# RajeshRk18/exacto

Measured on AMD Instinct MI355X. Metric: ciphertext muls/sec (bfv_mul_and_relin), higher is better.
Workload: dtype u64; 1 GPU; bfv_mul_and_relin, BASELINE configs[2]; ring_degree=4096, ct_limbs=3, limb_bits=60, plain_modulus=65537, gadget_base=65536, gadget_digits=12, batch_per_gpu=1024, global_batch=1024, parallelism=batch-shard x1

## Files before the change

### exacto_amd/csrc/ks32.hip

```cpp
#include "exacto_internal.hpp"
#include "ks32_dev.hpp"

#include <algorithm>

namespace exacto {


template <int LOGN, typename DT, int FORM>
__global__ void __launch_bounds__((1 << LOGN) / 16)
ks32_digit_ntt_kernel(const DT* __restrict__ D16, uint32_t* __restrict__ DS, int G, int S,
                      const Prime32* __restrict__ primes) {
    constexpr int N = 1 << LOGN, T = N / 16;
    __shared__ uint32_t lds[N];
    const int tid = threadIdx.x;
    const uint32_t b = blockIdx.x;
    const int s = (int)(b % (uint32_t)S);
    const long ig = b / (uint32_t)S;
    const Prime32& P = primes[s];
    const DT* src = D16 + ig * N;
    uint32_t x[16];
    constexpr bool SIN = FORM == F32_LAZY && sizeof(DT) == 2;
#pragma unroll
    for (int k = 0; k < 16; ++k) {
        const int d = src[tid + k * T];
// ... 46 lines not shown
    __syncthreads();
    for (int w = 128; w > 0; w >>= 1) {
        if ((int)threadIdx.x < w) part[threadIdx.x] += part[threadIdx.x + w];
        __syncthreads();
    }
    if (threadIdx.x == 0) out[row] = part[0];
}

__device__ __forceinline__ uint32_t red_s64(long long x, const Prime32& P) {
    const uint32_t p = P.p;
    const uint32_t hu = (uint32_t)((unsigned long long)x >> 32) ^ 0x80000000u;
    const uint32_t a = red32(shoup32(hu, P.c32, P.c32s, p), p);
    const uint32_t b = red32(red32((uint32_t)x, 2 * p), p);
    return red32(red32(a + b, p) + P.k63, p);
}

__device__ __forceinline__ uint32_t red_s64_lz(long long x, const Prime32& P) {
    const uint32_t p = P.p;
    const uint32_t hu = (uint32_t)((unsigned long long)x >> 32) ^ 0x80000000u;
    const uint32_t a = red32(shoup32(hu, P.c32, P.c32s, p), p);
    const uint32_t lo = (uint32_t)x;
    const uint32_t b = lo - (lo >> 30) * p;
    const uint32_t s = a + b + P.k63;
    return min(s, s - 2 * p);
}

__device__ __forceinline__ long long red_s64_lazy(long long x, const Prime32& P) {
    const uint32_t hu = (uint32_t)((unsigned long long)x >> 32) ^ 0x80000000u;
    const uint32_t a = shoup32(hu, P.c32, P.c32s, P.p);
    return (long long)((unsigned long long)a + (uint32_t)x + P.k63);
}

constexpr int KS_LS = 64;
template <int CLB, int NW, int RUN, bool LZ = false>
__global__ void __launch_bounds__(NW * 64)
ks32_mac_kernel(const int* __restrict__ DS, const int* __restrict__ RS, uint32_t* __restrict__ U,
                int G, int CL, int S, int items, int n, const Prime32* __restrict__ primes) {
    extern __shared__ int kl[];
    constexpr int IG = 4 * NW;
    const int lane = threadIdx.x & (KS_LS - 1);
    const int wave = __builtin_amdgcn_readfirstlane(threadIdx.x / KS_LS);
    const int nb = n / KS_LS;
    const int jb = blockIdx.x % nb;
    const int s = (blockIdx.x / nb) % S;
    const int cl0 = (blockIdx.x / (nb * S)) * CLB;
    const int j = jb * KS_LS + lane;
    const Prime32& P = primes[s];
    for (int rr = wave; rr < G * CLB; rr += NW) {
        const int g = rr / CLB, c = rr - g * CLB;
        kl[rr * KS_LS + lane] = RS[(((long)g * CL + cl0 + c) * S + s) * n + jb * KS_LS + lane];
    }
    __syncthreads();
    const int it_end = min(items, (int)(blockIdx.y + 1) * IG);
    for (int it = blockIdx.y * IG + wave; it < it_end; it += NW) {
        const int* dp = DS + ((long)it * G * S + s) * n + j;
        long long acc[CLB];
#pragma unroll
        for (int c = 0; c < CLB; ++c) acc[c] = 0;
        for (int g0 = 0; g0 < G; g0 += RUN) {
            int d[RUN];
#pragma unroll
            for (int e = 0; e < RUN; ++e) d[e] = dp[(long)min(g0 + e, G - 1) * S * n];
#pragma unroll
            for (int e = 0; e < RUN; ++e) d[e] = g0 + e < G ? d[e] : 0;
#pragma unroll
            for (int e = 0; e < RUN; ++e) {
                const int* kg = kl + (min(g0 + e, G - 1) * CLB) * KS_LS + lane;
#pragma unroll
                for (int c = 0; c < CLB; ++c) acc[c] += (long long)d[e] * kg[c * KS_LS];
            }
            if (g0 + RUN < G) {
#pragma unroll
                for (int c = 0; c < CLB; ++c) acc[c] = red_s64_lazy(acc[c], P);
            }
        }
#pragma unroll
        for (int c = 0; c < CLB; ++c)
            U[(((long)it * CL + cl0 + c) * S + s) * n + j] = LZ ? red_s64_lz(acc[c], P) : red_s64(acc[c], P);
    }
}

template <int LOGN, int S, bool LAZY, bool FPC>
__global__ void __launch_bounds__((1 << LOGN) / 16)
ks32_crt_kernel(const uint32_t* __restrict__ U, u64* __restrict__ R, long r_stride, int L,
                const Ks32Tables* __restrict__ KT, const Prime32* __restrict__ primes,
                const PrimeConst* __restrict__ qprimes) {
    constexpr int N = 1 << LOGN, T = N / 16;
    __shared__ uint32_t lds[N];
    const int tid = threadIdx.x;
    const uint32_t b = blockIdx.x;
    u64 x[16];
    ks32_crt_values<LOGN, S, LAZY, FPC>(x, U, R, r_stride, L, b, lds, tid, KT, primes, qprimes);
    const uint32_t CL = 2 * L;
    const long item = b / CL;
    const __amdgpu_buffer_rsrc_t rd = poly_rsrc(R + item * r_stride + (long)(b - (uint32_t)item * CL) * N, N * 8);
#pragma unroll
    for (int k = 0; k < 16; ++k) buf_st64(rd, x[k], tid * 8, k * T * 8);
}

template <typename OT, typename IT>
__global__ void __launch_bounds__(256)
ks32_digit_sum_kernel(const IT* __restrict__ D, int npairs, const int* __restrict__ term_start,
                      const CombineTerm* __restrict__ terms, OT* __restrict__ out, int d, int gu, int n,
                      int nsh) {
    const uint32_t row = blockIdx.x >> nsh;
    const int j = (int)(blockIdx.x & ((1u << nsh) - 1)) * 2048 + 8 * threadIdx.x;
    const uint32_t g = row % (uint32_t)gu;
    const uint32_t ik = row / (uint32_t)gu;
    const int k = (int)(ik % (uint32_t)d);
    const long item = ik / (uint32_t)d;
    int acc[8] = {0, 0, 0, 0, 0, 0, 0, 0};
    for (int t = term_start[k]; t < term_start[k + 1]; ++t) {
        const IT* src = D + ((item * npairs + terms[t].pair) * gu + g) * (long)n + j;
        if constexpr (sizeof(IT) == 2) {
            const uint4 w = *reinterpret_cast<const uint4*>(src);
            const uint32_t v[4] = {w.x, w.y, w.z, w.w};
#pragma unroll
            for (int h = 0; h < 4; ++h) {
                acc[2 * h] += (int)(int16_t)(v[h] & 0xFFFF);
                acc[2 * h + 1] += (int)(int16_t)(v[h] >> 16);
            }
        } else {
            const uint2 w = *reinterpret_cast<const uint2*>(src);
            const uint32_t v[2] = {w.x, w.y};
#pragma unroll
            for (int h = 0; h < 8; ++h) acc[h] += (int)(int8_t)(v[h >> 2] >> (8 * (h & 3)));
        }
    }
    if constexpr (sizeof(OT) == 2) {
        uint4 o;
        uint32_t* op = &o.x;
#pragma unroll
// ... 8 lines not shown


#define FORM_SWITCH(form, CALL)                          \
    switch (form) {                                      \
        case F32_LAZY: CALL(F32_LAZY); break;            \
        case F32_NARROW: CALL(F32_NARROW); break;        \
        default: CALL(F32_WIDE); break;                  \
    }

template <int LOGN>
static void ks32_launch_digits(const void* D, bool wide, uint32_t* DS, int items, int G, int S, const Prime32* primes,
                               int form, hipStream_t st) {
    const dim3 grid((unsigned)((long)items * G * S)), block((1 << LOGN) / 16);
#define DIG_(F_)                                                                                                \
    do {                                                                                                        \
        if (wide)                                                                                               \
            EXACTO_LAUNCH((ks32_digit_ntt_kernel<LOGN, int32_t, F_>), grid, block, 0, st, (const int32_t*)D, \
                               DS, G, S, primes);                                                               \
        else                                                                                                    \
            EXACTO_LAUNCH((ks32_digit_ntt_kernel<LOGN, int16_t, F_>), grid, block, 0, st, (const int16_t*)D, \
                               DS, G, S, primes);                                                               \
    } while (0)
    FORM_SWITCH(form, DIG_)
#undef DIG_
}

template <int LOGN>
static void ks32_launch_key(const u64* K, uint32_t* RS, long rows, int L, int S, const Prime32* primes,
                            const PrimeConst* qprimes, int form, hipStream_t st) {
#define KEY_(F_) EXACTO_LAUNCH((ks32_key_kernel<LOGN, F_>), dim3((unsigned)(rows * S)), dim3((1 << LOGN) / 16), 0, \
                                    st, K, RS, L, S, primes, qprimes)
    FORM_SWITCH(form, KEY_)
#undef KEY_
}

template <int LOGN, bool LAZY>
static void ks32_launch_crt(const uint32_t* U, u64* R, long r_stride, int items, int L, int S, const Ks32Tables* KT,
                            const Prime32* primes, const PrimeConst* qprimes, hipStream_t st, bool fpc) {
    const dim3 grid((unsigned)((long)items * 2 * L)), block((1 << LOGN) / 16);
#define CRT_(S_, F_) EXACTO_LAUNCH((ks32_crt_kernel<LOGN, S_, LAZY, F_>), grid, block, 0, st, U, R, r_stride, L, KT, \
                                   primes, qprimes)
    if (S == 2) {
        if (fpc) CRT_(2, true); else CRT_(2, false);
    } else if (S == 3) {
        if (fpc) CRT_(3, true); else CRT_(3, false);
    } else {
        if (fpc) CRT_(4, true); else CRT_(4, false);
    }
#undef CRT_
}

#define KS32_SWITCH(logn, CALL)                  \
    switch (logn) {                              \
        case 10: CALL(10); break;                \
        case 11: CALL(11); break;                \
        case 12: CALL(12); break;                \
        case 13: CALL(13); break;                \
        case 14: CALL(14); break;                \
        default: break;                          \
    }

void ks32_digits(const int16_t* D16, uint32_t* DS, int items, int G, int S, int logn, const Prime32* primes, int form,
                 hipStream_t st) {
    if (items <= 0) return;
#define CALL(L_) ks32_launch_digits<L_>(D16, false, DS, items, G, S, primes, form, st)
    KS32_SWITCH(logn, CALL)
#undef CALL
}

void ks32_digits32(const int32_t* D, uint32_t* DS, int items, int G, int S, int logn, const Prime32* primes, int form,
                   hipStream_t st) {
    if (items <= 0) return;
#define CALL(L_) ks32_launch_digits<L_>(D, true, DS, items, G, S, primes, form, st)
    KS32_SWITCH(logn, CALL)
#undef CALL
}

void ks32_key(const u64* K, uint32_t* RS, long rows, int L, int S, int logn, const Prime32* primes,
              const PrimeConst* qprimes, int form, hipStream_t st) {
    if (rows <= 0) return;
#define CALL(L_) ks32_launch_key<L_>(K, RS, rows, L, S, primes, qprimes, form, st)
    KS32_SWITCH(logn, CALL)
#undef CALL
}

void ks32_key_norms(const u64* K, u64* out, long rows, int L, int n, const PrimeConst* qprimes, hipStream_t st) {
    if (rows <= 0) return;
    EXACTO_LAUNCH(ks32_key_norm_kernel, dim3((unsigned)rows), dim3(256), 0, st, K, out, L, n, qprimes);
}

void ks32_mac(const uint32_t* DS, const uint32_t* RS, uint32_t* U, int items, int G, int L, int S, int n,
              const Prime32* primes, int mac_form, hipStream_t st) {
    if (items <= 0) return;
    const int CL = 2 * L;
    int CLB = CL;
    while (CLB > 1 && (CL % CLB != 0 || (size_t)G * CLB * KS_LS * sizeof(int) > 65536)) --CLB;
    const size_t lds = (size_t)G * CLB * KS_LS * sizeof(int);
    const int NW = lds > 32768 ? 8 : 4;
    const dim3 grid((unsigned)((n / KS_LS) * S * (CL / CLB)), (unsigned)((items + 4 * NW - 1) / (4 * NW)));
    const int* ds = reinterpret_cast<const int*>(DS);
    const int* rs = reinterpret_cast<const int*>(RS);
#define MAC_(C_, W_, R_, Z_) EXACTO_LAUNCH((ks32_mac_kernel<C_, W_, R_, Z_>), grid, dim3(W_ * 64), lds, st, ds, rs, U, G, CL, S, items, n, primes)
#define MAC(C_)                                                  \
    do {                                                         \
        if (mac_form == 2) { if (NW == 8) MAC_(C_, 8, 12, true); else MAC_(C_, 4, 12, true); } \
        else if (mac_form == 1) { if (NW == 8) MAC_(C_, 8, 12, false); else MAC_(C_, 4, 12, false); } \
        else { if (NW == 8) MAC_(C_, 8, 7, false); else MAC_(C_, 4, 7, false); }          \
    } while (0)
    switch (CLB) {
        case 8: MAC(8); break;
        case 6: MAC(6); break;
        case 4: MAC(4); break;
        case 3: MAC(3); break;
        case 2: MAC(2); break;
        default: MAC(1); break;
    }
#undef MAC
#undef MAC_
}

void ks32_digit_sum(const void* D, bool in8, int npairs, const int* term_start, const CombineTerm* terms, void* out,
                    bool wide, int items, int d, int gu, int n, hipStream_t st) {
    const long rows = (long)items * d * gu;
    if (rows <= 0) return;
    const int nb = n >= 2048 ? n / 2048 : 1;
    const dim3 grid((unsigned)(rows * nb)), block(n >= 2048 ? 256 : n / 8);
    const int nsh = __builtin_ctz((unsigned)nb);
#define DSUM_(OT, IT) EXACTO_LAUNCH((ks32_digit_sum_kernel<OT, IT>), grid, block, 0, st, (const IT*)D, npairs, \
                                         term_start, terms, (OT*)out, d, gu, n, nsh)
    if (wide) {
        if (in8) DSUM_(int32_t, int8_t); else DSUM_(int32_t, int16_t);
    } else {
        if (in8) DSUM_(int16_t, int8_t); else DSUM_(int16_t, int16_t);
    }
#undef DSUM_
}

void ks32_crt(const uint32_t* U, u64* R, long r_stride, int items, int L, int S, int logn, const Ks32Tables* KT,
              const Prime32* primes, const PrimeConst* qprimes, int form, hipStream_t st, bool fpc) {
    if (items <= 0) return;
    fpc = fpc && (S <= 3 || form != F32_WIDE);
#define CALL(L_)                                                                                                \
    do {                                                                                                        \
        if (form == F32_LAZY) ks32_launch_crt<L_, true>(U, R, r_stride, items, L, S, KT, primes, qprimes, st, fpc); \
        else ks32_launch_crt<L_, false>(U, R, r_stride, items, L, S, KT, primes, qprimes, st, fpc);                \
    } while (0)
    KS32_SWITCH(logn, CALL)
#undef CALL
}

}
```

### exacto_amd/csrc/context.hip

```cpp
#include <algorithm>
#include <cxxabi.h>
#include <dlfcn.h>
#include <chrono>
#include <condition_variable>
#include <cmath>
#include <cstdio>
#include <cstdlib>
#include <cstring>
#include <functional>
#include <map>
#include <memory>
#include <mutex>
#include <set>
#include <string>
#include <thread>
#include <vector>

#include "../../include/exacto_hip.h"
#include "exacto_internal.hpp"

using namespace exacto;

thread_local const void* exacto::g_last_kernel = nullptr;

// ... 1098 lines not shown
        if (hipEventRecord(rec.b, c->stream) == hipSuccess) c->recs.push_back(rec);
    }
};

static int run_ntt(exacto_ctx* c, const NttBatch& nb, long count, bool inverse) {
    if (count <= 0) return 0;
    ProfScope ps(c, inverse ? PK_INV : PK_FWD, (u64)count, ((nb.src16 ? 2.0 : 8.0) + 8.0) * c->n * (double)count);
    bool lazy = true, near60 = c->ntt_asm;
    int qbits = 0;
    for (int t = nb.prime_base; t < nb.prime_base + nb.period; ++t) {
        lazy &= c->primes[t] < (1ull << 60);
        near60 &= c->primes[t] < (1ull << 60) && c->primes[t] > (1ull << 60) - (1ull << 32);
        qbits = std::max(qbits, 64 - __builtin_clzll(c->primes[t]));
    }
    launch_ntt(nb, (int)count, c->logn, inverse, lazy, c->d_primes, c->stream, near60, near60 && c->ntt_asm_inv, qbits);
    CHECK_LAUNCH();
    return 0;
}

static int run_ntt_fwd2(exacto_ctx* c, const NttBatch& nb1, long count1, const NttBatch& nb2, long count2) {
    bool near60 = c->ntt_asm && !nb1.src16 && !nb2.src16;
    for (u64 q : c->primes) near60 &= q < (1ull << 60) && q > (1ull << 60) - (1ull << 32);
    if (near60 && count1 > 0 && count2 > 0) {
        ProfScope ps(c, PK_FWD, (u64)(count1 + count2), 16.0 * c->n * (double)(count1 + count2));
        if (launch_ntt_fwd2(nb1, (int)count1, nb2, (int)count2, c->logn, c->d_primes, c->stream)) {
            CHECK_LAUNCH();
            return 0;
        }
    }
    if (int e = run_ntt(c, nb1, count1, false)) return e;
    return run_ntt(c, nb2, count2, false);
}

static bool tensor_asm(const exacto_ctx* c) {
    bool near60 = c->ntt_asm && c->ntt_asm_inv;
    for (int t = 0; t < c->L + c->K; ++t)
        near60 &= c->primes[t] < (1ull << 60) && c->primes[t] > (1ull << 60) - (1ull << 24);
    return near60;
}

static int run_inv_tensor(exacto_ctx* c, const Operands& o, int cnt, bool p2only = false) {
    const int NP = c->L + c->K;
    bool lazy = true;
    const bool near60 = tensor_asm(c);
    int qbits = 0;
    for (int t = 0; t < NP; ++t) {
        qbits = std::max(qbits, 64 - __builtin_clzll(c->primes[t]));
        lazy &= c->primes[t] < (1ull << 60);
    }
    const double pb = 8.0 * c->n;
    double bytes;
    if (c->tensor_share_d > 0 && c->tensor_share_npairs > 0) {
        const double items = (double)((cnt + c->tensor_share_npairs - 1) / c->tensor_share_npairs);
        const double cts = items * 2.0 * c->tensor_share_d;
        bytes = pb * (c->L * (2.0 * cts + 3.0 * cnt) +
                      c->K * (p2only ? cts + (double)cnt : 2.0 * cts + 3.0 * cnt));
    } else {
        bytes = cnt * (p2only ? pb * (7.0 * c->L + 3.0 * c->K) : pb * 7.0 * NP);
    }
    ProfScope ps(c, PK_TENSOR, (u64)cnt * (p2only ? 3 * c->L + c->K : 3 * NP), bytes);
    launch_inv_tensor(o, c->ws_extP, c->ws_T, cnt, c->logn, c->L, c->K, lazy, c->d_primes, c->stream, near60, p2only,
                      qbits, c->tensor_share_npairs, near60 && c->path != EXACTO_PATH_HPS);
    CHECK_LAUNCH();
    return 0;
}

// ... 282 lines not shown
        if (c->path == EXACTO_PATH_HPS) {
            void* d16p = hps_defer ? (c->ks_defer8 ? (void*)((int8_t*)c->ks_defer + s * (long)guse * n)
                                                   : (void*)(c->ks_defer + s * (long)guse * n))
                                   : nullptr;
            launch_hps_scale(c->ws_T, R, out_stride, ncomp, hps_defer ? nullptr : D, d16p,
                             hps_defer && c->ks_defer8, guse, cnt, n, c->d_crt, c->d_primes, K, c->hps_fast,
                             c->stream);
        } else
            launch_exact_scale(c->ws_T, R, out_stride, ncomp, d16 ? nullptr : D,
                               d16 ? (c->ks_defer ? (c->ks_defer8
                                                         ? (int16_t*)((int8_t*)c->ks_defer + s * (long)guse * n)
                                                         : c->ks_defer + s * (long)guse * n)
                                                  : c->ws_D16)
                                   : nullptr,
                               guse, cnt, n, c->d_crt, c->d_primes, L, K, crt_mode(c),
                               c->stream, c->h_crt.gshift, ps.on, c->ks_defer && c->ks_defer8, c->fp_crt, c->fpq_lim);
        CHECK_LAUNCH();
        }
        if (ps.on) {
            const long item0 = s / ps.npairs;
            const double ib = (double)(cnt / ps.npairs);
            ProfScope pq(c, PK_PSUM_SCALE, (u64)(cnt / ps.npairs) * ps.d,
                         ib * 2.0 * n * 8.0 * (ps.d * (double)(K + L) + (double)ps.npairs * L));
            if (!launch_psum_scale(c->ws_T, c->ws_extP, ps.out + item0 * ps.d * 2 * Ln, cnt / ps.npairs, ps.d, ps.npairs,
                                   ps.term_start, ps.terms, n, c->d_crt, c->d_primes, L, c->stream, ps.fpc,
                                   c->fpq_lim))
                return fail(EXACTO_ERR_HIP, "internal: psum scale not available for these limbs");
            CHECK_LAUNCH();
        }
        NttBatch rb{};
        rb.src = R; rb.src_off = nullptr; rb.src_item_stride = out_stride;
        rb.dst = R; rb.dst_item_stride = out_stride;
        rb.ppi = ncomp * L; rb.prime_base = 0; rb.period = L;
        if (k32) {
            if (!c->ks_defer) {
                {
                    ProfScope pd(c, PK_KS_DIGITS, (u64)cnt * guse * c->S32, 6.0 * n * cnt * guse * c->S32);
                    ks32_digits(c->ws_D16, c->ws_DS, cnt, guse, c->S32, c->logn, c->d_p32, c->ks32_mac_form, c->stream);
                }
                {
                    ProfScope pm(c, PK_KS_MAC, (u64)cnt * c->S32, 4.0 * n * cnt * c->S32 * (guse + 2.0 * L));
                    ks32_mac(c->ws_DS, c->d_rs, c->ws_U, cnt, guse, L, c->S32, n, c->d_p32, c->ks32_mac_form, c->stream);
                }
                {
                    ProfScope pc(c, PK_KS_CRT, (u64)cnt * 2 * L, (double)n * cnt * 2 * L * (4.0 * c->S32 + 16.0));
                    ks32_crt(c->ws_U, R, out_stride, cnt, L, c->S32, c->logn, c->d_kst, c->d_p32, c->d_primes, c->ks32_mac_form,
                             c->stream, c->ks_fpc && c->ks32_fpc_max >= 1);
                }
                CHECK_LAUNCH();
            }
        }
        if (skip_fwd) continue;
        if (int e = run_ntt(c, rb, (long)cnt * ncomp * L, false)) return e;
        if (relin && guse > 0 && !k32) {
            NttBatch db = contiguous(c->ws_D, cnt, (long)guse * L, 0, L, n);
            if (d16) {
                db.src16 = c->ws_D16;
                db.src16_item_stride = (long)guse * n;
            }
            if (int e = run_ntt(c, db, (long)cnt * guse * L, false)) return e;
            if (int e = ensure_rlk_companions(c)) return e;
            {
                ProfScope pm(c, PK_RELIN_MAC, (u64)cnt, 8.0 * n * L * cnt * (4.0 + guse));
                launch_relin_mac(R, out_stride, c->ws_D, c->d_rlk, c->d_rlk_s, guse, R, out_stride, cnt, n, L,
                                 c->d_primes, c->stream);
            }
            CHECK_LAUNCH();
        }
    }
    return 0;
}


static int check_ctx(exacto_ctx* c) {
    if (!c) return invalid_param("null context");
    HIP_TRY(hipSetDevice(c->device));
    return 0;
}

static int ntt_dev(exacto_ctx* c, uint64_t* polys, size_t count, size_t limb, bool inverse) {
    if (int e = check_ctx(c)) return e;
    if (limb >= (size_t)c->L)
        return fail(EXACTO_ERR_DIMENSION_MISMATCH, "dimension mismatch: expected " + std::to_string(c->L) + ", got " +
                                                       std::to_string(limb));
    return run_ntt(c, contiguous(polys, count, 1, (int)limb, 1, c->n), (long)count, inverse);
}
// ... 1129 lines not shown
        if (e) return e;
    } else {
        size_t cap = c->gk_s_cap;
        if (grow(&c->gk_s, &cap, count * sizeof(u64))) return EXACTO_ERR_HIP;
        c->gk_s_cap = cap;
        launch_shoup_companions(gk, c->gk_s, (long)count, n, L, c->d_primes, c->stream);
        CHECK_LAUNCH();
    }
    const size_t C = std::min<size_t>(c->chunk, B);
    if (int e = ensure_workspace(c, C)) return e;
    int nl = 1;
    if (int e = fork_lanes(c, (long)((B + C - 1) / C), C, &nl)) return e;
    LaneJoin join{c, nl};
    for (size_t s0 = 0; s0 < B; s0 += C) {
        const int cnt = (int)std::min(C, B - s0);
        LaneGuard lane(c, (int)((s0 / C) % (size_t)nl));
        const u64* src = ct + s0 * 2 * Ln;
        u64* dst = out + s0 * 2 * Ln;
        NttBatch nb{};
        nb.src = src; nb.src_item_stride = 2 * Ln;
        nb.dst = c->ws_coefQ; nb.dst_item_stride = 2 * Ln;
        nb.ppi = 2 * L; nb.prime_base = 0; nb.period = L;
        if (int e = run_ntt(c, nb, (long)cnt * 2 * L, true)) return e;
        launch_automorph(c->ws_coefQ, 2 * Ln, c->ws_T, 2 * Ln, cnt, 2, n, L, element, c->d_primes, -1, c->stream);
        CHECK_LAUNCH();
        if (k32) {
            launch_decompose(c->ws_T + Ln, 2 * Ln, c->ws_D, guse, cnt, n, c->d_crt, c->d_primes, L, c->stream,
                             c->ws_D16);
            CHECK_LAUNCH();
            launch_rows(c->ws_T + Ln, 2 * Ln, nullptr, 0, Ln, cnt, c->stream);
            CHECK_LAUNCH();
            ks32_digits(c->ws_D16, c->ws_DS, cnt, guse, kb.S, c->logn, kb.d_p32, kb.mac_form, c->stream);
            ks32_mac(c->ws_DS, c->d_gk_rs, c->ws_U, cnt, guse, L, kb.S, n, kb.d_p32, kb.mac_form, c->stream);
            ks32_crt(c->ws_U, c->ws_T, 2 * Ln, cnt, L, kb.S, c->logn, kb.d_kst, kb.d_p32, c->d_primes, kb.mac_form, c->stream,
                     c->ks_fpc && kb.fpc_max >= 1);
            CHECK_LAUNCH();
            NttBatch rb{};
            rb.src = c->ws_T; rb.src_item_stride = 2 * Ln;
            rb.dst = dst; rb.dst_item_stride = 2 * Ln;
            rb.ppi = 2 * L; rb.prime_base = 0; rb.period = L;
            if (int e = run_ntt(c, rb, (long)cnt * 2 * L, false)) return e;
            continue;
        }
        NttBatch c0{};
        c0.src = c->ws_T; c0.src_item_stride = 2 * Ln;
        c0.dst = dst; c0.dst_item_stride = 2 * Ln;
        c0.ppi = L; c0.prime_base = 0; c0.period = L;
        if (int e = run_ntt(c, c0, (long)cnt * L, false)) return e;
        launch_rows(dst + Ln, 2 * Ln, nullptr, 0, Ln, cnt, c->stream);
        launch_decompose(c->ws_T + Ln, 2 * Ln, c->ws_D, guse, cnt, n, c->d_crt, c->d_primes, L, c->stream,
                         d16 ? c->ws_D16 : nullptr);
        CHECK_LAUNCH();
        NttBatch db = contiguous(c->ws_D, cnt, (long)guse * L, 0, L, n);
        if (d16) {
            db.src16 = c->ws_D16;
            db.src16_item_stride = (long)guse * n;
        }
        if (int e = run_ntt(c, db, (long)cnt * guse * L, false)) return e;
        launch_relin_mac(dst, 2 * Ln, c->ws_D, gk, c->gk_s, guse, dst, 2 * Ln, cnt, n, L, c->d_primes, c->stream);
        CHECK_LAUNCH();
    }
    return 0;
}

extern "C" int exacto_gen_galois_key(exacto_ctx* c, const uint64_t* sk, uint64_t element, double sigma,
                                     const uint64_t* key, uint64_t stream, size_t num_keys, uint64_t* gk) {
    if (!c) return invalid_param("null context");
    return host_call(c, {{sk, c->L * poly_bytes(c)}}, num_keys * 2 * c->L * poly_bytes(c), gk,
                     [&](std::vector<u64*>& d, u64* o) {
// ... 1371 lines not shown
```

### exacto_amd/csrc/exacto_internal.hpp

```cpp
#pragma once
#include "arith.hpp"

namespace exacto {

struct NttBatch {
    const u64* src;
    const u64* src_off;
    long src_item_stride;
    u64* dst;
    long dst_item_stride;
    int ppi;
    int prime_base;
    int period;
    const int16_t* src16;
    long src16_item_stride;
    int lazy_out;
};

enum class MulPath : int { Exact = 0, Hps = 1 };

struct CrtTables {
    int L;
    int K;
    int G;
// ... 49 lines not shown

#define EXACTO_KS32_MAXS 4
struct Prime32 {
    uint32_t p;
    uint32_t n_inv, n_inv_s;
    uint32_t last_w, last_ws;
    uint32_t c32, c32s;
    uint32_t k63;
    uint32_t fn_inv, fn_inv_s;
    uint32_t flast_w, flast_ws;
    double inv_p;
    const uint2* tw_fwd;
    const uint2* tw_inv;
};
struct Ks32Tables {
    uint32_t ginv[EXACTO_KS32_MAXS][EXACTO_KS32_MAXS];
    uint32_t ginv_s[EXACTO_KS32_MAXS][EXACTO_KS32_MAXS];
    uint32_t halfP[EXACTO_KS32_MAXS];
    u64 pref_w[EXACTO_MAX_L][EXACTO_KS32_MAXS];
    u64 pref_ws[EXACTO_MAX_L][EXACTO_KS32_MAXS];
    u64 negP[EXACTO_MAX_L];
    uint32_t fpc_c[EXACTO_MAX_L][EXACTO_KS32_MAXS][2];
    uint32_t fpc_n[EXACTO_MAX_L][2];
};
void ks32_digits(const int16_t* D16, uint32_t* DS, int items, int G, int S, int logn, const Prime32* primes,
                 int form, hipStream_t st);
void ks32_digits32(const int32_t* D, uint32_t* DS, int items, int G, int S, int logn, const Prime32* primes,
                   int form, hipStream_t st);
void ks32_key(const u64* K, uint32_t* RS, long rows, int L, int S, int logn, const Prime32* primes,
              const PrimeConst* qprimes, int form, hipStream_t st);
void ks32_key_norms(const u64* K, u64* out, long rows, int L, int n, const PrimeConst* qprimes, hipStream_t st);
void ks32_mac(const uint32_t* DS, const uint32_t* RS, uint32_t* U, int items, int G, int L, int S, int n,
              const Prime32* primes, int mac_form, hipStream_t st);
void ks32_crt(const uint32_t* U, u64* R, long r_stride, int items, int L, int S, int logn, const Ks32Tables* KT,
              const Prime32* primes, const PrimeConst* qprimes, int form, hipStream_t st, bool fpc = false);

struct Operands {
    const u64* a;
    const u64* a_off;
    long a_stride;
    const u64* b;
    const u64* b_off;
    long b_stride;
    const u64* ea;
    const u64* ea_off;
    const u64* eb;
    const u64* eb_off;
};

bool launch_polymul(const u64* A, const u64* B, u64* out, long rows, int period, int logn, const PrimeConst* primes,
                    hipStream_t s);
void launch_mul_inv(const u64* A, const u64* B, u64* out, long rows, int period, int logn, bool lazy, bool asm_inv,
                    const PrimeConst* primes, hipStream_t s);
void launch_inv_tensor(const Operands& op, const u64* extP, u64* T, int items, int logn, int L, int K, bool lazy,
                       const PrimeConst* primes, hipStream_t s, bool asm_inv = false, bool p2only = false,
                       int qbits = 64, int share_np = 0, bool lazy_out = false);
void launch_phase(const u64* ct, int polys, long ct_stride, const u64* sk, u64* out, int items, int n, int L,
                  const PrimeConst* primes, hipStream_t s);
void launch_decrypt_round(const u64* X, u64* out, int items, int n, int L, const CrtTables* ct,
                          const PrimeConst* primes, u64 plain, hipStream_t s);
void launch_dbfv_recompose(const u64* digits, u64* out, int items, int n, int d, u64 base, u64 plain, u64 t,
                           bool scalar, hipStream_t s);
void launch_exact_lift(const u64* coefQ, u64* extP, long rows, int n, const CrtTables* ct,
                       const PrimeConst* primes, int L, int K, int mode, hipStream_t s);
void launch_hps_extend(const u64* coefQ, u64* extP, long rows, int n, const PrimeConst* primes,
                       int K, hipStream_t s);
bool exact_scale_sp_ok(int L, int K, int mode);
void launch_exact_scale(const u64* T, u64* R, long r_stride, int ncomp_r, u64* D, int16_t* D16, int guse,
// ... 90 lines not shown
```

### exacto_amd/csrc/ntt.hip

```cpp
#include "exacto_internal.hpp"
#include "ks32_dev.hpp"
#include "bufmem.hpp"
#include "crt_dev.hpp"

namespace exacto {

#ifndef EXACTO_TW_AS
#define EXACTO_TW_AS 1
#endif
#if EXACTO_TW_AS == 0
typedef const TwPair* TwTab;
#else
typedef const TwPair __attribute__((address_space(EXACTO_TW_AS)))* TwTab;
#endif

__device__ __forceinline__ TwTab tw_table(const TwPair* p) { return (TwTab)p; }

__device__ __forceinline__ TwPair ld_tw(TwTab tab, int i) {
    TwPair t;
    t.w = tab[i].w;
    t.ws = tab[i].ws;
    return t;
}

// ... 591 lines not shown
#undef PIN_SYN
    } else if (nb.src16) {
        const int16_t* s16 = nb.src16 + (long)item * nb.src16_item_stride + (long)(sub / nb.period) * N + tid;
#define PIN_IN16(k) { const i64 d_ = s16[(k) * T]; PIN_SET(k, d_ < 0 ? q + (u64)d_ : (u64)d_) }
        PIN_X16(PIN_IN16)
#undef PIN_IN16
    } else {
        const u64* src = nb.src + (nb.src_off ? (long)nb.src_off[item] : (long)item * nb.src_item_stride) +
                         (long)sub * N;
        const PolyRd rs(src, N * 8);
#define PIN_IN64(k) PIN_SET(k, rs.ld64(tid * 8, (k) * T * 8))
        PIN_X16(PIN_IN64)
#undef PIN_IN64
    }
    if constexpr (PROBE == 2) {
        PIN_EXCHANGE(lds, tid, LOGN - 4, LOGN - 8)
        PIN_EXCHANGE(lds, tid, LOGN - 8, LOGN == 12 ? 0 : 1)
        if constexpr (LOGN == 13) {
            if constexpr (EXACTO_FWD13_LP) EXACTO_XCHG_PIN_LP(tid);
            else PIN_EXCHANGE(lds, tid, 1, 0)
        }
    } else if constexpr (LZO) {
        PIN_FWD_ROUNDS(LOGN, lds, tid, tw_table(P.tw_fwd), make_asmk(q), _LZ)
    } else {
        PIN_FWD_ROUNDS(LOGN, lds, tid, tw_table(P.tw_fwd), make_asmk(q), )
    }
    if constexpr (PROBE == 1) {
        if (nb.dst_item_stride != -7) return;
    }
    const PolyWr rd(dst, N * 8);
#define PIN_OUT(k) rd.st64(PIN_GET(k), tid * 8, fwd_pin_value_of_home<LOGN>(k) * T * 8);
    PIN_X16(PIN_OUT)
#undef PIN_OUT
}


__device__ __forceinline__ u64 barrett_mul_lazy(u64 a, u64 b, const PrimeConst& P) {
    const u64 hi = __umul64hi(a, b), lo = a * b;
    const int s = P.bar_s;
    const u64 xs = (lo >> (s - 1)) | (hi << (65 - s));
    const u64 qhat = ((xs * P.bar_mu) >> (s + 1)) | (__umul64hi(xs, P.bar_mu) << (63 - s));
    return lo - qhat * P.q;
}

__device__ __forceinline__ u64 mulmod_near60(u64 a, u64 b, uint32_t d) {
    constexpr u64 M60 = (1ull << 60) - 1;
    const u64 lo = a * b, hi = __umul64hi(a, b);
    const u64 H = (hi << 4) | (lo >> 60);
    const u64 xl = (lo & M60) + (u64)(uint32_t)H * d;
    const u64 xh = (u64)(uint32_t)(H >> 32) * d + (xl >> 32);
    const u64 H2 = xh >> 28;
    const u64 L2 = ((xh & 0x0FFFFFFFull) << 32) | (uint32_t)xl;
    return L2 + H2 * d;
}

#ifndef EXACTO_MUL_ASM
#define EXACTO_MUL_ASM 1
#endif
template <bool ASM = (EXACTO_MUL_ASM != 0)>
__device__ __forceinline__ void mul2_near60(u64& r0, u64 a0, u64 b0, u64& r1, u64 a1, u64 b1, uint32_t d) {
    if constexpr (ASM) {
        MulNear60Asm<2>::run(r0, r1, a0, b0, a1, b1, d, 16 * d);
    } else {
        r0 = mulmod_near60(a0, b0, d);
        r1 = mulmod_near60(a1, b1, d);
    }
// ... 515 lines not shown
    if (share_np < 8 || items % share_np != 0) share_np = 0;
    const long blocks = (long)items * 3 * (L + K);
    if (blocks == 0) return;
    if (p2only) {
        if (logn == 12) launch_it<12>(op, extP, T, blocks, L, K, lazy, primes, s, true, 1, 64, share_np, lazy_out);
        else if (logn == 13) launch_it<13>(op, extP, T, blocks, L, K, lazy, primes, s, true, 1, 64, share_np, lazy_out);
        return;
    }
    switch (logn) {
        case 4: launch_it<4>(op, extP, T, blocks, L, K, lazy, primes, s); break;
        case 5: launch_it<5>(op, extP, T, blocks, L, K, lazy, primes, s); break;
        case 6: launch_it<6>(op, extP, T, blocks, L, K, lazy, primes, s); break;
        case 7: launch_it<7>(op, extP, T, blocks, L, K, lazy, primes, s); break;
        case 8: launch_it<8>(op, extP, T, blocks, L, K, lazy, primes, s); break;
        case 9: launch_it<9>(op, extP, T, blocks, L, K, lazy, primes, s); break;
        case 10: launch_it<10>(op, extP, T, blocks, L, K, lazy, primes, s, false, 0, qbits, share_np); break;
        case 11: launch_it<11>(op, extP, T, blocks, L, K, lazy, primes, s); break;
        case 12: launch_it<12>(op, extP, T, blocks, L, K, lazy, primes, s, asm_inv, 0, qbits, share_np, lazy_out); break;
        case 13: launch_it<13>(op, extP, T, blocks, L, K, lazy, primes, s, asm_inv, 0, qbits, share_np, lazy_out); break;
        case 14: launch_it<14>(op, extP, T, blocks, L, K, lazy, primes, s); break;
        default: break;
    }
}

bool launch_ntt_fwd2(const NttBatch& nb1, int count1, const NttBatch& nb2, int count2, int logn,
                     const PrimeConst* primes, hipStream_t s) {
    if (count1 <= 0 || count2 <= 0 || (logn != 12 && logn != 13)) return false;
    const dim3 grid((unsigned)(count1 + count2));
    if (logn == 12) EXACTO_LAUNCH((ntt_fwd_pin_kernel<12>), grid, dim3(256), 0, s, nb1, primes, nb2, count1);
    else EXACTO_LAUNCH((ntt_fwd_pin_kernel<13>), grid, dim3(512), 0, s, nb1, primes, nb2, count1);
    return true;
}

void launch_ntt(const NttBatch& nb, int count, int logn, bool inverse, bool lazy, const PrimeConst* primes,
                hipStream_t s, bool asm_fwd, bool asm_inv, int qbits) {
    if (count <= 0) return;
    if (asm_fwd && !inverse && (logn == 12 || logn == 13)) {
        if (nb.lazy_out) {
            if (logn == 12) EXACTO_LAUNCH((ntt_fwd_pin_kernel<12, 0, true>), dim3(count), dim3(256), 0, s, nb, primes);
            else EXACTO_LAUNCH((ntt_fwd_pin_kernel<13, 0, true>), dim3(count), dim3(512), 0, s, nb, primes);
        } else {
            if (logn == 12) EXACTO_LAUNCH((ntt_fwd_pin_kernel<12>), dim3(count), dim3(256), 0, s, nb, primes);
            else EXACTO_LAUNCH((ntt_fwd_pin_kernel<13>), dim3(count), dim3(512), 0, s, nb, primes);
        }
        return;
    }
    if (asm_inv && inverse && (logn == 12 || logn == 13)) {
        if (logn == 12) EXACTO_LAUNCH((ntt_inv_pin_kernel<12>), dim3(count), dim3(256), 0, s, nb, primes);
        else EXACTO_LAUNCH((ntt_inv_pin_kernel<13>), dim3(count), dim3(512), 0, s, nb, primes);
        return;
    }
    if (lazy && (logn == 10 || logn == 12 || logn == 13) && ntt_gen_on()) {
        const dim3 th(1u << (logn - 4));
#define GEN_NTT_(K_, LG_, QB_) EXACTO_LAUNCH((K_<LG_, QB_>), dim3(count), th, 0, s, nb, primes)
        if (inverse) {
            if (logn == 10) { if (gen_small<10>(qbits)) GEN_NTT_(ntt_inv_gen_kernel, 10, 50); else GEN_NTT_(ntt_inv_gen_kernel, 10, 60); }
            else if (logn == 12) { if (gen_small<12>(qbits)) GEN_NTT_(ntt_inv_gen_kernel, 12, 56); else GEN_NTT_(ntt_inv_gen_kernel, 12, 60); }
            else GEN_NTT_(ntt_inv_gen_kernel, 13, 60);
        } else {
            if (logn == 10) { if (gen_small<10>(qbits)) GEN_NTT_(ntt_fwd_gen_kernel, 10, 50); else GEN_NTT_(ntt_fwd_gen_kernel, 10, 60); }
            else if (logn == 12) { if (gen_small<12>(qbits)) GEN_NTT_(ntt_fwd_gen_kernel, 12, 56); else GEN_NTT_(ntt_fwd_gen_kernel, 12, 60); }
            else GEN_NTT_(ntt_fwd_gen_kernel, 13, 60);
        }
#undef GEN_NTT_
        return;
    }
// ... 25 lines not shown
```

Measured before the change: 481,800 bfv_mul_and_relin/s.

## Software-pipeline key-switch MAC digit loads and batch key staging via buffer loads

Restructures the key-switch MAC kernel so each wave double-buffers its digit loads, fetching the next run or item while multiplying the current one, and collapses the item and digit loops into one state machine. Key rows are staged into LDS in batches of nine buffer loads per wave, and all global accesses use buffer resources. The host picks the items-per-block adaptively so the grid has at least twice the CU count of blocks. A specialised single-run variant drops the loop when all digits fit in one run. The change adds register pressure and code complexity in exchange for hiding global memory latency.

Result: no change. 483,200 bfv_mul_and_relin/s (median of 6 runs) (+0.3%).

```diff
diff --git a/exacto_amd/csrc/ks32.hip b/exacto_amd/csrc/ks32.hip
--- a/exacto_amd/csrc/ks32.hip
+++ b/exacto_amd/csrc/ks32.hip
@@ -102,52 +102,88 @@
 }
 
 constexpr int KS_LS = 64;
-template <int CLB, int NW, int RUN, bool LZ = false>
+constexpr unsigned KS_CUS = 256;
+constexpr int KS_SB = 9;
+template <int CLB, int NW, int RUN, bool LZ, bool ONE>
 __global__ void __launch_bounds__(NW * 64)
 ks32_mac_kernel(const int* __restrict__ DS, const int* __restrict__ RS, uint32_t* __restrict__ U,
-                int G, int CL, int S, int items, int n, const Prime32* __restrict__ primes) {
+                int G, int CL, int S, int items, int IG, int n, const Prime32* __restrict__ primes) {
     extern __shared__ int kl[];
-    constexpr int IG = 4 * NW;
     const int lane = threadIdx.x & (KS_LS - 1);
     const int wave = __builtin_amdgcn_readfirstlane(threadIdx.x / KS_LS);
     const int nb = n / KS_LS;
     const int jb = blockIdx.x % nb;
     const int s = (blockIdx.x / nb) % S;
     const int cl0 = (blockIdx.x / (nb * S)) * CLB;
-    const int j = jb * KS_LS + lane;
+    const int j0 = jb * KS_LS;
+    const int voff = lane * 4;
+    const int rowb = n * 4;
     const Prime32& P = primes[s];
-    for (int rr = wave; rr < G * CLB; rr += NW) {
-        const int g = rr / CLB, c = rr - g * CLB;
-        kl[rr * KS_LS + lane] = RS[(((long)g * CL + cl0 + c) * S + s) * n + jb * KS_LS + lane];
+    {
+        const int rows = G * CLB;
+        const __amdgpu_buffer_rsrc_t rk =
+            poly_rsrc(RS + ((long)cl0 * S + s) * n + j0, (((G - 1) * CL + CLB - 1) * S * n + KS_LS) * 4);
+        for (int r0 = wave; r0 < rows; r0 += NW * KS_SB) {
+            int v[KS_SB];
+#pragma unroll
+            for (int k = 0; k < KS_SB; ++k) {
+                const int rr = min(r0 + k * NW, rows - 1);
+                const int g = rr / CLB, c = rr - g * CLB;
+                v[k] = (int)buf_ld32(rk, voff, (g * CL + c) * S * rowb);
+            }
+#pragma unroll
+            for (int k = 0; k < KS_SB; ++k) kl[min(r0 + k * NW, rows - 1) * KS_LS + lane] = v[k];
+        }
     }
     __syncthreads();
     const int it_end = min(items, (int)(blockIdx.y + 1) * IG);
-    for (int it = blockIdx.y * IG + wave; it < it_end; it += NW) {
-        const int* dp = DS + ((long)it * G * S + s) * n + j;
-        long long acc[CLB];
-#pragma unroll
-        for (int c = 0; c < CLB; ++c) acc[c] = 0;
-        for (int g0 = 0; g0 < G; g0 += RUN) {
-            int d[RUN];
-#pragma unroll
-            for (int e = 0; e < RUN; ++e) d[e] = dp[(long)min(g0 + e, G - 1) * S * n];
-#pragma unroll
-            for (int e = 0; e < RUN; ++e) d[e] = g0 + e < G ? d[e] : 0;
-#pragma unroll
-            for (int e = 0; e < RUN; ++e) {
-                const int* kg = kl + (min(g0 + e, G - 1) * CLB) * KS_LS + lane;
-#pragma unroll
-                for (int c = 0; c < CLB; ++c) acc[c] += (long long)d[e] * kg[c * KS_LS];
+    const int it0 = blockIdx.y * IG + wave;
+    if (it0 >= it_end) return;
+    const int dsz = ((G - 1) * S * n + KS_LS) * 4;
+    const int usz = ((CLB - 1) * S * n + KS_LS) * 4;
+    auto load_run = [&](int (&b)[RUN], int it, int g0) {
+        const __amdgpu_buffer_rsrc_t rd = poly_rsrc(DS + ((long)it * G * S + s) * n + j0, dsz);
+#pragma unroll
+        for (int e = 0; e < RUN; ++e) b[e] = (int)buf_ld32(rd, voff, min(g0 + e, G - 1) * S * rowb);
+    };
+    long long acc[CLB];
+#pragma unroll
+    for (int c = 0; c < CLB; ++c) acc[c] = 0;
+    int it = it0, g0 = 0;
+    auto step = [&](int (&cb)[RUN], int (&nb)[RUN]) -> bool {
+        const bool more = !ONE && g0 + RUN < G;
+        const bool last = it + NW >= it_end;
+        const int nit = more || last ? it : it + NW, ng0 = more ? g0 + RUN : 0;
+        load_run(nb, nit, ng0);
+        __builtin_amdgcn_sched_barrier(0);
+        int kofs = lane;
+        asm volatile("" : "+v"(kofs));
+#pragma unroll
+        for (int e = 0; e < RUN; ++e) {
+            const int* kg = kl + min(g0 + e, G - 1) * CLB * KS_LS + kofs;
+            const int d = g0 + e < G ? cb[e] : 0;
+#pragma unroll
+            for (int c = 0; c < CLB; ++c) acc[c] += (long long)d * kg[c * KS_LS];
+        }
+        if (more) {
+#pragma unroll
+            for (int c = 0; c < CLB; ++c) acc[c] = red_s64_lazy(acc[c], P);
+        } else {
+            const __amdgpu_buffer_rsrc_t ru = poly_rsrc(U + (((long)it * CL + cl0) * S + s) * n + j0, usz);
+#pragma unroll
+            for (int c = 0; c < CLB; ++c) {
+                buf_st32(ru, LZ ? red_s64_lz(acc[c], P) : red_s64(acc[c], P), voff, c * S * rowb);
+                acc[c] = 0;
             }
-            if (g0 + RUN < G) {
-#pragma unroll
-                for (int c = 0; c < CLB; ++c) acc[c] = red_s64_lazy(acc[c], P);
-            }
+            if (last) return false;
         }
-#pragma unroll
-        for (int c = 0; c < CLB; ++c)
-            U[(((long)it * CL + cl0 + c) * S + s) * n + j] = LZ ? red_s64_lz(acc[c], P) : red_s64(acc[c], P);
-    }
+        it = nit;
+        g0 = ng0;
+        return true;
+    };
+    int da[RUN], db[RUN];
+    load_run(da, it0, 0);
+    while (step(da, db) && step(db, da)) {}
 }
 
 template <int LOGN, int S, bool LAZY, bool FPC>
@@ -307,15 +343,23 @@
     while (CLB > 1 && (CL % CLB != 0 || (size_t)G * CLB * KS_LS * sizeof(int) > 65536)) --CLB;
     const size_t lds = (size_t)G * CLB * KS_LS * sizeof(int);
     const int NW = lds > 32768 ? 8 : 4;
-    const dim3 grid((unsigned)((n / KS_LS) * S * (CL / CLB)), (unsigned)((items + 4 * NW - 1) / (4 * NW)));
+    const unsigned gx = (unsigned)((n / KS_LS) * S * (CL / CLB));
+    int IG = 16 * NW;
+    while (IG > 4 * NW && gx * (unsigned)((items + IG - 1) / IG) < 2 * KS_CUS) IG /= 2;
+    const dim3 grid(gx, (unsigned)((items + IG - 1) / IG));
     const int* ds = reinterpret_cast<const int*>(DS);
     const int* rs = reinterpret_cast<const int*>(RS);
-#define MAC_(C_, W_, R_, Z_) EXACTO_LAUNCH((ks32_mac_kernel<C_, W_, R_, Z_>), grid, dim3(W_ * 64), lds, st, ds, rs, U, G, CL, S, items, n, primes)
+#define MAC__(C_, W_, R_, Z_, O_) EXACTO_LAUNCH((ks32_mac_kernel<C_, W_, R_, Z_, O_>), grid, dim3(W_ * 64), lds, st, ds, rs, U, G, CL, S, items, IG, n, primes)
+#define MAC_(C_, R_, Z_)                                         \
+    do {                                                         \
+        if (G <= R_) { if (NW == 8) MAC__(C_, 8, R_, Z_, true); else MAC__(C_, 4, R_, Z_, true); } \
+        else { if (NW == 8) MAC__(C_, 8, R_, Z_, false); else MAC__(C_, 4, R_, Z_, false); }       \
+    } while (0)
 #define MAC(C_)                                                  \
     do {                                                         \
-        if (mac_form == 2) { if (NW == 8) MAC_(C_, 8, 12, true); else MAC_(C_, 4, 12, true); } \
-        else if (mac_form == 1) { if (NW == 8) MAC_(C_, 8, 12, false); else MAC_(C_, 4, 12, false); } \
-        else { if (NW == 8) MAC_(C_, 8, 7, false); else MAC_(C_, 4, 7, false); }          \
+        if (mac_form == 2) MAC_(C_, 12, true);                   \
+        else if (mac_form == 1) MAC_(C_, 12, false);             \
+        else MAC_(C_, 7, false);                                 \
     } while (0)
     switch (CLB) {
         case 8: MAC(8); break;
@@ -327,6 +371,7 @@
     }
 #undef MAC
 #undef MAC_
+#undef MAC__
 }
 
 void ks32_digit_sum(const void* D, bool in8, int npairs, const int* term_start, const CombineTerm* terms, void* out,
```

## Fuse forward NTT into ks32 CRT kernel for keyswitch output

Applied to the files above, without the earlier changes.

Moves the ks32 CRT kernel into the NTT source and adds a variant that runs the pinned forward-NTT rounds on the CRT-reconstructed values in registers before storing. Relinearization and Galois keyswitch paths pass a destination so the separate forward NTT launch is skipped when the fused variant applies. This removes one global-memory round trip of the output polynomials and one kernel launch. In exchange it raises register pressure and LDS size, uses a waves-per-EU hint, and falls back when S or the lazy form does not fit.

Result: no change. 488,000 bfv_mul_and_relin/s before, 492,500 bfv_mul_and_relin/s after (median of 6 runs) (+0.9%).

```diff
diff --git a/exacto_amd/csrc/context.hip b/exacto_amd/csrc/context.hip
--- a/exacto_amd/csrc/context.hip
+++ b/exacto_amd/csrc/context.hip
@@ -1154,6 +1154,13 @@
     return run_ntt(c, nb2, count2, false);
 }
 
+static bool ntt_fwd_pinned(const exacto_ctx* c, int prime_base, int period) {
+    bool near60 = c->ntt_asm && (c->logn == 12 || c->logn == 13);
+    for (int t = prime_base; t < prime_base + period; ++t)
+        near60 &= c->primes[t] < (1ull << 60) && c->primes[t] > (1ull << 60) - (1ull << 32);
+    return near60;
+}
+
 static bool tensor_asm(const exacto_ctx* c) {
     bool near60 = c->ntt_asm && c->ntt_asm_inv;
     for (int t = 0; t < c->L + c->K; ++t)
@@ -1502,8 +1509,10 @@
         rb.src = R; rb.src_off = nullptr; rb.src_item_stride = out_stride;
         rb.dst = R; rb.dst_item_stride = out_stride;
         rb.ppi = ncomp * L; rb.prime_base = 0; rb.period = L;
+        bool fwd_done = false;
         if (k32) {
             if (!c->ks_defer) {
+                const bool fuse = !skip_fwd && ntt_fwd_pinned(c, 0, L);
                 {
                     ProfScope pd(c, PK_KS_DIGITS, (u64)cnt * guse * c->S32, 6.0 * n * cnt * guse * c->S32);
                     ks32_digits(c->ws_D16, c->ws_DS, cnt, guse, c->S32, c->logn, c->d_p32, c->ks32_mac_form, c->stream);
@@ -1514,14 +1523,16 @@
                 }
                 {
                     ProfScope pc(c, PK_KS_CRT, (u64)cnt * 2 * L, (double)n * cnt * 2 * L * (4.0 * c->S32 + 16.0));
-                    ks32_crt(c->ws_U, R, out_stride, cnt, L, c->S32, c->logn, c->d_kst, c->d_p32, c->d_primes, c->ks32_mac_form,
-                             c->stream, c->ks_fpc && c->ks32_fpc_max >= 1);
+                    fwd_done = ks32_crt(c->ws_U, R, out_stride, cnt, L, c->S32, c->logn, c->d_kst, c->d_p32, c->d_primes,
+                                        c->ks32_mac_form, c->stream, c->ks_fpc && c->ks32_fpc_max >= 1,
+                                        fuse ? R : nullptr, out_stride);
                 }
                 CHECK_LAUNCH();
             }
         }
         if (skip_fwd) continue;
-        if (int e = run_ntt(c, rb, (long)cnt * ncomp * L, false)) return e;
+        if (!fwd_done)
+            if (int e = run_ntt(c, rb, (long)cnt * ncomp * L, false)) return e;
         if (relin && guse > 0 && !k32) {
             NttBatch db = contiguous(c->ws_D, cnt, (long)guse * L, 0, L, n);
             if (d16) {
@@ -2717,9 +2728,11 @@
             CHECK_LAUNCH();
             ks32_digits(c->ws_D16, c->ws_DS, cnt, guse, kb.S, c->logn, kb.d_p32, kb.mac_form, c->stream);
             ks32_mac(c->ws_DS, c->d_gk_rs, c->ws_U, cnt, guse, L, kb.S, n, kb.d_p32, kb.mac_form, c->stream);
-            ks32_crt(c->ws_U, c->ws_T, 2 * Ln, cnt, L, kb.S, c->logn, kb.d_kst, kb.d_p32, c->d_primes, kb.mac_form, c->stream,
-                     c->ks_fpc && kb.fpc_max >= 1);
+            const bool fwd_done = ks32_crt(c->ws_U, c->ws_T, 2 * Ln, cnt, L, kb.S, c->logn, kb.d_kst, kb.d_p32, c->d_primes,
+                                           kb.mac_form, c->stream, c->ks_fpc && kb.fpc_max >= 1,
+                                           ntt_fwd_pinned(c, 0, L) ? dst : nullptr, 2 * Ln);
             CHECK_LAUNCH();
+            if (fwd_done) continue;
             NttBatch rb{};
             rb.src = c->ws_T; rb.src_item_stride = 2 * Ln;
             rb.dst = dst; rb.dst_item_stride = 2 * Ln;
diff --git a/exacto_amd/csrc/exacto_internal.hpp b/exacto_amd/csrc/exacto_internal.hpp
--- a/exacto_amd/csrc/exacto_internal.hpp
+++ b/exacto_amd/csrc/exacto_internal.hpp
@@ -105,8 +105,9 @@
 void ks32_key_norms(const u64* K, u64* out, long rows, int L, int n, const PrimeConst* qprimes, hipStream_t st);
 void ks32_mac(const uint32_t* DS, const uint32_t* RS, uint32_t* U, int items, int G, int L, int S, int n,
               const Prime32* primes, int mac_form, hipStream_t st);
-void ks32_crt(const uint32_t* U, u64* R, long r_stride, int items, int L, int S, int logn, const Ks32Tables* KT,
-              const Prime32* primes, const PrimeConst* qprimes, int form, hipStream_t st, bool fpc = false);
+bool ks32_crt(const uint32_t* U, u64* R, long r_stride, int items, int L, int S, int logn, const Ks32Tables* KT,
+              const Prime32* primes, const PrimeConst* qprimes, int form, hipStream_t st, bool fpc = false,
+              u64* fwd_dst = nullptr, long fwd_stride = 0);
 
 struct Operands {
     const u64* a;
diff --git a/exacto_amd/csrc/ks32.hip b/exacto_amd/csrc/ks32.hip
--- a/exacto_amd/csrc/ks32.hip
+++ b/exacto_amd/csrc/ks32.hip
@@ -150,24 +150,6 @@
     }
 }
 
-template <int LOGN, int S, bool LAZY, bool FPC>
-__global__ void __launch_bounds__((1 << LOGN) / 16)
-ks32_crt_kernel(const uint32_t* __restrict__ U, u64* __restrict__ R, long r_stride, int L,
-                const Ks32Tables* __restrict__ KT, const Prime32* __restrict__ primes,
-                const PrimeConst* __restrict__ qprimes) {
-    constexpr int N = 1 << LOGN, T = N / 16;
-    __shared__ uint32_t lds[N];
-    const int tid = threadIdx.x;
-    const uint32_t b = blockIdx.x;
-    u64 x[16];
-    ks32_crt_values<LOGN, S, LAZY, FPC>(x, U, R, r_stride, L, b, lds, tid, KT, primes, qprimes);
-    const uint32_t CL = 2 * L;
-    const long item = b / CL;
-    const __amdgpu_buffer_rsrc_t rd = poly_rsrc(R + item * r_stride + (long)(b - (uint32_t)item * CL) * N, N * 8);
-#pragma unroll
-    for (int k = 0; k < 16; ++k) buf_st64(rd, x[k], tid * 8, k * T * 8);
-}
-
 template <typename OT, typename IT>
 __global__ void __launch_bounds__(256)
 ks32_digit_sum_kernel(const IT* __restrict__ D, int npairs, const int* __restrict__ term_start,
@@ -242,22 +224,6 @@
                                     st, K, RS, L, S, primes, qprimes)
     FORM_SWITCH(form, KEY_)
 #undef KEY_
-}
-
-template <int LOGN, bool LAZY>
-static void ks32_launch_crt(const uint32_t* U, u64* R, long r_stride, int items, int L, int S, const Ks32Tables* KT,
-                            const Prime32* primes, const PrimeConst* qprimes, hipStream_t st, bool fpc) {
-    const dim3 grid((unsigned)((long)items * 2 * L)), block((1 << LOGN) / 16);
-#define CRT_(S_, F_) EXACTO_LAUNCH((ks32_crt_kernel<LOGN, S_, LAZY, F_>), grid, block, 0, st, U, R, r_stride, L, KT, \
-                                   primes, qprimes)
-    if (S == 2) {
-        if (fpc) CRT_(2, true); else CRT_(2, false);
-    } else if (S == 3) {
-        if (fpc) CRT_(3, true); else CRT_(3, false);
-    } else {
-        if (fpc) CRT_(4, true); else CRT_(4, false);
-    }
-#undef CRT_
 }
 
 #define KS32_SWITCH(logn, CALL)                  \
@@ -346,17 +312,4 @@
 #undef DSUM_
 }
 
-void ks32_crt(const uint32_t* U, u64* R, long r_stride, int items, int L, int S, int logn, const Ks32Tables* KT,
-              const Prime32* primes, const PrimeConst* qprimes, int form, hipStream_t st, bool fpc) {
-    if (items <= 0) return;
-    fpc = fpc && (S <= 3 || form != F32_WIDE);
-#define CALL(L_)                                                                                                \
-    do {                                                                                                        \
-        if (form == F32_LAZY) ks32_launch_crt<L_, true>(U, R, r_stride, items, L, S, KT, primes, qprimes, st, fpc); \
-        else ks32_launch_crt<L_, false>(U, R, r_stride, items, L, S, KT, primes, qprimes, st, fpc);                \
-    } while (0)
-    KS32_SWITCH(logn, CALL)
-#undef CALL
-}
-
-}
+}
diff --git a/exacto_amd/csrc/ntt.hip b/exacto_amd/csrc/ntt.hip
--- a/exacto_amd/csrc/ntt.hip
+++ b/exacto_amd/csrc/ntt.hip
@@ -647,6 +647,44 @@
 #define PIN_OUT(k) rd.st64(PIN_GET(k), tid * 8, fwd_pin_value_of_home<LOGN>(k) * T * 8);
     PIN_X16(PIN_OUT)
 #undef PIN_OUT
+}
+
+
+template <int LOGN, int S, bool LAZY, bool FPC, bool FWD = false>
+__global__ void __launch_bounds__((1 << LOGN) / 16) __attribute__((amdgpu_waves_per_eu(FWD ? 4 : 0)))
+ks32_crt_kernel(const uint32_t* __restrict__ U, const u64* R, long r_stride, u64* D, long d_stride, int L,
+                const Ks32Tables* __restrict__ KT, const Prime32* __restrict__ primes,
+                const PrimeConst* __restrict__ qprimes) {
+    constexpr int N = 1 << LOGN, T = N / 16;
+    __shared__ u64 lds64[FWD ? N : N / 2];
+    uint32_t* lds = reinterpret_cast<uint32_t*>(lds64);
+    const int tid = threadIdx.x;
+    const uint32_t b = blockIdx.x;
+    u64 x[16];
+    ks32_crt_values<LOGN, S, LAZY, FPC>(x, U, R, r_stride, L, b, lds, tid, KT, primes, qprimes);
+    const uint32_t CL = 2 * L;
+    const long item = b / CL;
+    const int cl = (int)(b - (uint32_t)item * CL);
+    u64* dst = D + item * d_stride + (long)cl * N;
+    if constexpr (!FWD) {
+        const __amdgpu_buffer_rsrc_t rd = poly_rsrc(dst, N * 8);
+#pragma unroll
+        for (int k = 0; k < 16; ++k) buf_st64(rd, x[k], tid * 8, k * T * 8);
+    } else {
+        static_assert(LOGN == 12 || LOGN == 13, "pinned rounds exist for n = 4096 and 8192");
+        const PrimeConst& P = qprimes[cl % L];
+        int tf = tid;
+        asm volatile("" : "+v"(tf));
+        EXACTO_PIN_DECL
+#define PIN_INX(k) PIN_SET(k, x[k])
+        PIN_X16(PIN_INX)
+#undef PIN_INX
+        PIN_FWD_ROUNDS(LOGN, lds64, tf, tw_table(P.tw_fwd), make_asmk(P.q), )
+        const PolyWr rd(dst, N * 8);
+#define PIN_OUT(k) rd.st64(PIN_GET(k), tf * 8, fwd_pin_value_of_home<LOGN>(k) * T * 8);
+        PIN_X16(PIN_OUT)
+#undef PIN_OUT
+    }
 }
 
 
@@ -1228,6 +1266,65 @@
     return true;
 }
 
+#ifndef EXACTO_KS_CRT_FWD
+#define EXACTO_KS_CRT_FWD 1
+#endif
+
+template <int LOGN, int S, bool LAZY>
+constexpr bool ks32_crt_fwd_fits() { return S == 3 || (S == 4 && (LOGN == 13 || !LAZY)); }
+
+template <int LOGN, bool LAZY, bool FWD>
+static bool ks32_launch_crt(const uint32_t* U, const u64* R, long r_stride, u64* D, long d_stride, int items, int L,
+                            int S, const Ks32Tables* KT, const Prime32* primes, const PrimeConst* qprimes,
+                            hipStream_t st, bool fpc) {
+    const dim3 grid((unsigned)((long)items * 2 * L)), block((1 << LOGN) / 16);
+#define CRT_(S_, F_)                                                                                              \
+    do {                                                                                                          \
+        if constexpr (!FWD || ks32_crt_fwd_fits<LOGN, S_, LAZY>())                                                \
+            EXACTO_LAUNCH((ks32_crt_kernel<LOGN, S_, LAZY, F_, FWD>), grid, block, 0, st, U, R, r_stride, D,      \
+                          d_stride, L, KT, primes, qprimes);                                                      \
+        else                                                                                                      \
+            return false;                                                                                         \
+    } while (0)
+    if (S == 2) {
+        if (fpc) CRT_(2, true); else CRT_(2, false);
+    } else if (S == 3) {
+        if (fpc) CRT_(3, true); else CRT_(3, false);
+    } else {
+        if (fpc) CRT_(4, true); else CRT_(4, false);
+    }
+#undef CRT_
+    return true;
+}
+
+bool ks32_crt(const uint32_t* U, u64* R, long r_stride, int items, int L, int S, int logn, const Ks32Tables* KT,
+              const Prime32* primes, const PrimeConst* qprimes, int form, hipStream_t st, bool fpc, u64* fwd_dst,
+              long fwd_stride) {
+    if (items <= 0) return false;
+    fpc = fpc && (S <= 3 || form != F32_WIDE);
+    const bool lazy = form == F32_LAZY;
+#define CALL(L_, Z_, W_)                                                                                          \
+    ks32_launch_crt<L_, Z_, W_>(U, R, r_stride, W_ ? fwd_dst : R, W_ ? fwd_stride : r_stride, items, L, S, KT, primes, \
+                                qprimes, st, fpc)
+    if (EXACTO_KS_CRT_FWD && fwd_dst && (logn == 12 || logn == 13)) {
+        const bool done = logn == 12 ? (lazy ? CALL(12, true, true) : CALL(12, false, true))
+                                     : (lazy ? CALL(13, true, true) : CALL(13, false, true));
+        if (done) return true;
+    }
+#define CALL2(L_) do { if (lazy) CALL(L_, true, false); else CALL(L_, false, false); } while (0)
+    switch (logn) {
+        case 10: CALL2(10); break;
+        case 11: CALL2(11); break;
+        case 12: CALL2(12); break;
+        case 13: CALL2(13); break;
+        case 14: CALL2(14); break;
+        default: break;
+    }
+#undef CALL2
+#undef CALL
+    return false;
+}
+
 void launch_ntt(const NttBatch& nb, int count, int logn, bool inverse, bool lazy, const PrimeConst* primes,
                 hipStream_t s, bool asm_fwd, bool asm_inv, int qbits) {
     if (count <= 0) return;
```
